# vkit-x/vkit

Hardware: AMD Instinct MI355X
Metric: Mpixels/s (2048^2 RGB, geo+photo chain) (higher is better)
Workload: dtype u8; 1 GPU; C3 fused chain: camera_cubic_curve remap (level 5) + gaussian_blur(sigma=1.0) + color_shift(37) + gaussion_noise(std=10.0, the numpy stream default_rng(5000 + i) drawn on the device inside every step), states built from the configs inside every step, 2048x2048x3 uint8, batch 256 per GPU; batch_per_gpu=256, image=2048x2048x3, noise_mode=tiles, states=built on the device from the configs inside every step (vkx_camera_states_dev), lanes=1

## Files before the change

### vkit_amd/csrc/fused.hip

```cpp
#include "vkx_internal.h"
#include "vkx_cell.h"
#include "vkx_color.h"

#include <float.h>
#include <memory>
#include <stdlib.h>
#include <string.h>

namespace {

constexpr int W = 64;
constexpr int RMAX = 3;
constexpr int NLDSCELL = 64;
#ifndef VKX_FUSED_NWAVES
#define VKX_FUSED_NWAVES 8
#endif
constexpr int NWAVES = VKX_FUSED_NWAVES;
constexpr int NTHREADS = 64 * NWAVES;
constexpr int ROWS_PER_WAVE = 8;
constexpr int WH = NWAVES * ROWS_PER_WAVE;
__host__ __device__ constexpr int tile_side(int R) { return (W - 2 * R) & ~3; }
__host__ __device__ constexpr int tile_height(int R) { return WH == W ? tile_side(R) : WH - 2 * R; }
#ifndef VKX_FUSED_CGROUP
#define VKX_FUSED_CGROUP 2
// ... 25 lines not shown
    int R;
    int hue_on, hue_delta;
    unsigned short kq[8];
    int streak_on, streak_step, streak_thickness, streak_dash, streak_dash_step, streak_dash_gap;
    int streak_vert, streak_hori, streak_copy;
    int streak_color[3];
    float streak_alpha;
    int n_elems, pad_;
    const uint2 *noise_table;
    int noise_tiled, noise_tiles, noise_slot;
    float noise_tiles_per_sample;
    const uint2 *noise_rows;
    struct Elem {
        const void *src;
        void *dst;
        ptrdiff_t sstride, dstride;
        int cn, is_f32;
    } el[4];
};

struct ElemPack {
    ItemDev::Elem el[4];
    int n;
};

struct TileRect {
    int x0, y0, x1, y1;
    __host__ __device__ bool empty() const { return x1 < x0 || y1 < y0; }
};
__host__ __device__ inline TileRect interior_rect(int dw, int dh, int R)
{
    const int Tw = tile_side(R), Th = tile_height(R);
    TileRect r;
    r.x0 = (R + Tw - 1) / Tw;
    r.y0 = (R + Th - 1) / Th;
    r.x1 = dw - W + R >= 0 ? (dw - W + R) / Tw : -1;
    r.y1 = dh - WH + R >= 0 ? (dh - WH + R) / Th : -1;
    return r;
}

struct TileBin {
    int rmin, cmin;
    int rmax1, cmax1;
};

struct CellR {
    int ex[4], edx[4];
    short vx[4], vy[4];
    int flags, pad;
};
static_assert(sizeof(CellR) == 56, "CellR mirrors the tail of CellC");

__device__ __forceinline__ int find_item(const int *__restrict__ prefix, int n, int v)
{
    int lo = 0, hi = n - 1;
    while (lo < hi) {
        const int mid = (lo + hi + 1) >> 1;
        if (prefix[mid] <= v) lo = mid; else hi = mid - 1;
    }
    return lo;
}

constexpr int kLocalBins = 1024;

__global__ void __launch_bounds__(256) k_chain_setup(const ItemDev *__restrict__ items, const int *__restrict__ cell_prefix,
                                                     int n_items, int total_cells, int slots,
                                                     vkc::CellC *__restrict__ cells, TileBin *__restrict__ bins,
                                                     int *__restrict__ deferred )
{
    __shared__ int lbins[kLocalBins * 4];
// ... 436 lines not shown
                        px += ax + (step ? bx : 0);
                        py += ay + (step ? by : 0);
                    }
                } else {
                    const double h6 = lch[kk * 9 + 6], h7 = lch[kk * 9 + 7];
                    for (int s = k0; s <= k1; s++) {
                        const bool inside = (unsigned)(px - lox) < (unsigned)nx_ && (unsigned)(py - loy) < (unsigned)ny_;
                        if (inside && !(fma(1.0, 1.0, fma(h7, (double)(py + wy0), h6 * (double)(px + wx0))) == 0))
                            atomicMax(own + py * P_ + px, tag);
                        const bool step = err < 0;
                        err += step ? up : down;
                        px += ax + (step ? bx : 0);
                        py += ay + (step ? by : 0);
                    }
                }
            }
        }
        __syncthreads();
        if (phase_limit == 1) return;

        if (!INTERIOR && nc > NLDSCELL) {
            load_chunk(0, NLDSCELL);
            __syncthreads();
        }

        const int gx = wx0 + lane;
        const bool colok = INTERIOR || (gx >= cx0 && gx < cx1);
        int srcl[2 * RMAX + 1];
#pragma unroll
        for (int i = 0; i < 2 * RMAX + 1; i++) {
            int s = (R > 0 && i < K) ? (INTERIOR ? lane + i - R : vkd::reflect101(gx + i - R, dw) - wx0) : lane;
            srcl[i] = min(max(s, 0), W - 1) << 2;
        }
        const unsigned fast_xlim = (unsigned)max(sw - 2, 0), fast_ylim = (unsigned)max(sh - 1, 0);
        const double fxd = (double)gx;
        const bool exact_div = __builtin_amdgcn_readfirstlane(*lflag) != 0;
        for (int g0 = 0; g0 < ROWS_PER_WAVE; g0 += CGROUP) {
            int X[CGROUP], Y[CGROUP];
            bool rowok[CGROUP];
#pragma unroll
            for (int u = 0; u < CGROUP; u++) {
                const int ly = wave * ROWS_PER_WAVE + g0 + u;
                const int gy = wy0 + ly;
                rowok[u] = INTERIOR || (gy >= cy0 && gy < cy1);
                X[u] = 0; Y[u] = 0;
                if (rowok[u] && colok) {
                    const uint32_t o = own[ly * P_ + lane];
                    if (o != 0) {
                        const int k = (int)o - 1;
                        double h[8];
                        if (INTERIOR || k < NLDSCELL) {
                            lds_cdouble_t hp = (lds_cdouble_t)(lch + __umul24(k, 9));
                            asm volatile("" : "+v"(hp));
#pragma unroll
                            for (int j = 0; j < 8; j++) h[j] = hp[j];
                        } else {
                            const vkc::CellC VKX_GLOBAL *gc =
                                (const vkc::CellC VKX_GLOBAL *)(gcell + (r0 + div_small(k, ncol, rcp_ncol)) * cw + (c0 + k - div_small(k, ncol, rcp_ncol) * ncol));
#pragma unroll
                            for (int j = 0; j < 8; j++) h[j] = gc->H[j];
                        }
                        const double fy = (double)gy;
                        const double nx = fma(h[2], 1.0, fma(h[1], fy, h[0] * fxd));
                        const double ny = fma(h[5], 1.0, fma(h[4], fy, h[3] * fxd));
                        const double de = fma(1.0, 1.0, fma(h[7], fy, h[6] * fxd));
                        float qxf, qyf;
                        if (exact_div || !div_pair_f32_fast(nx, ny, de, qxf, qyf)) {
                            double qx, qy;
                            div_pair(nx, ny, de, qx, qy);
                            X[u] = vkd::cv_round((float)qx * 32.f);
                            Y[u] = vkd::cv_round((float)qy * 32.f);
                        } else {
                            X[u] = cvt_i32_sat(rintf(qxf * 32.f));
                            Y[u] = cvt_i32_sat(rintf(qyf * 32.f));
                        }
                    }
                }
            }
            if constexpr (KIND == 3) {
#pragma unroll
// ... 77 lines not shown
                    const uint32_t o0 = __umul24((uint32_t)sy, (uint32_t)sstride) + __umul24((uint32_t)sx, 3u);
                    ta[u] = *(const u64_u1 VKX_GLOBAL *)(src + (size_t)o0);
                    tb[u] = *(const u64_u1 VKX_GLOBAL *)(src + (size_t)(o0 + (uint32_t)sstride));
                }
            }
            uint32_t prb[CGROUP], pg[CGROUP];
#pragma unroll
            for (int u = 0; u < CGROUP; u++) {
                prb[u] = 0; pg[u] = 0;
                if (!rowok[u]) continue;
                if (colok) {
                    const int fx = X[u] & 31, fy = Y[u] & 31;
                    if (fast[u]) {
                        const uint32_t wx = (uint32_t)(32 - fx) | ((uint32_t)fx << 24);
                        const uint32_t t0 = (uint32_t)ta[u], t1 = (uint32_t)(ta[u] >> 32), b0 = (uint32_t)tb[u], b1 = (uint32_t)(tb[u] >> 32);
                        const uint32_t ar = __builtin_amdgcn_udot4(t0, wx, 0u, false);
                        const uint32_t ag = __builtin_amdgcn_udot4(__builtin_amdgcn_alignbyte(t1, t0, 1), wx, 0u, false);
                        const uint32_t ab = __builtin_amdgcn_udot4(__builtin_amdgcn_alignbyte(t1, t0, 2), wx, 0u, false);
                        const uint32_t br = __builtin_amdgcn_udot4(b0, wx, 0u, false);
                        const uint32_t bg = __builtin_amdgcn_udot4(__builtin_amdgcn_alignbyte(b1, b0, 1), wx, 0u, false);
                        const uint32_t bb = __builtin_amdgcn_udot4(__builtin_amdgcn_alignbyte(b1, b0, 2), wx, 0u, false);
                        const uint32_t wy0 = (uint32_t)(32 - fy), wy1 = (uint32_t)fy;
                        const uint32_t r = mad_u24(br, wy1, mad_u24_cs(ar, wy0, 512u)) >> 10;
                        const uint32_t g = mad_u24(bg, wy1, mad_u24_cs(ag, wy0, 512u)) >> 10;
                        const uint32_t b = mad_u24(bb, wy1, mad_u24_cs(ab, wy0, 512u)) >> 10;
                        prb[u] = r | (b << 16);
                        pg[u] = g;
                    } else {
                        rim_sample_rgb(src, sh, sw, sstride, X[u], Y[u], prb[u], pg[u]);
                    }
                }
            }
            static_assert(CGROUP == 2, "phase D works on the window-row pair of one iteration");
            const int ly0 = wave * ROWS_PER_WAVE + g0;
            if (!(rowok[0] || rowok[1])) continue;
            if (R > 0) {
                const uint32_t gg = pg[0] | (pg[1] << 16);
                uint32_t a0 = 0, a1 = 0, ag = 0;
#pragma unroll
                for (int i = 0; i < 2 * RMAX + 1; i++) {
                    if (i < K) {
                        uint32_t v0 = prb[0], v1 = prb[1], vg = gg;
                        if (!(INTERIOR && RC >= 0 && i == RC)) {
                            v0 = (uint32_t)__builtin_amdgcn_ds_bpermute(srcl[i], (int)prb[0]);
                            v1 = (uint32_t)__builtin_amdgcn_ds_bpermute(srcl[i], (int)prb[1]);
                            vg = (uint32_t)__builtin_amdgcn_ds_bpermute(srcl[i], (int)gg);
                        }
                        a0 = mad_u24_ks(kq[i], v0, a0);
                        a1 = mad_u24_ks(kq[i], v1, a1);
                        ag = mad_u24_ks(kq[i], vg, ag);
                    }
                }
                uint32_t *pl = own + ly0 * P_ + lane;
                pl[0] = __builtin_amdgcn_perm(a1, a0, 0x05040100u);
                pl[64] = ag;
                pl[128] = __builtin_amdgcn_perm(a1, a0, 0x07060302u);
            } else {
#pragma unroll
                for (int u = 0; u < CGROUP; u++)
                    if (rowok[u]) own[(ly0 + u) * P_ + lane] = (prb[u] & 0xffu) | (pg[u] << 8) | (prb[u] & 0xff0000u);
            }
        }
        if constexpr (KIND == 3) return;
        __syncthreads();
        if (phase_limit == 2) return;

    }
// ... 703 lines not shown
```

### vkit_amd/csrc/nprand.hip

```cpp
#include "vkx_internal.h"
#include "np_ziggurat.h"
#include "vkx_host_tables.h"

#include <stddef.h>
#include <string.h>
#include <algorithm>

namespace {

typedef unsigned __int128 u128;
#define VKX_GLOBAL __attribute__((address_space(1)))

#ifndef VKX_NP_ROUNDS
#define VKX_NP_ROUNDS 48
#endif
constexpr int kRounds = VKX_NP_ROUNDS;
static_assert(kRounds % 2 == 0 && kRounds >= 2 && kRounds <= 64, "rounds per tile");
constexpr int kTile = 64 * kRounds;
constexpr double kNorR = 3.6541528853610087963519472518;
constexpr double kNorInvR = 0.27366123732975827203338247596;

#define PCG_MULT VKX_PCG_MULT
using vkx_host_tables::JumpTabs;

struct NpTabs {
    JumpTabs jump;
    uint64_t ki[256], wi[256], fi[256];
};

struct NpJob {
    uint64_t state[2], inc[2];
    uint64_t c64[2];
    uint64_t c128[2];
    long long n;
    long long tile_base;
    int n_tiles;
    int kind, cn;
    double loc, scale;
    double margin;
    double cdf[3];
    const uint8_t *src;
    void *dst;
    int16_t *rec;
    uint2 *table;
};

struct TileInfo {
    uint32_t count0, out0;
    uint64_t start0, emit0;
};
constexpr uint32_t kIrregular = 0x80000000u;
constexpr uint32_t kParkOver = 0x40000000u;
constexpr uint32_t kOutCarry = 0x3fffffffu;
constexpr uint32_t kFlagParkOver = 0x40000000u;
struct TilePlan {
    unsigned long long prefix;
    uint32_t c_in, count;
};

typedef uint32_t u32x4 __attribute__((ext_vector_type(4)));
struct FiC { double fi, c; };
__device__ __forceinline__ u128 mk128(const uint64_t *w) { return ((u128)w[1] << 64) | (u128)w[0]; }

__device__ __forceinline__ uint64_t pcg_out(u128 s)
{
    const uint64_t hi = (uint64_t)(s >> 64), lo = (uint64_t)s;
    const uint64_t x = hi ^ lo;
    const unsigned r = (unsigned)(hi >> 58);
    return (x >> r) | (x << ((64 - r) & 63));
}
struct LcgStride {
    uint32_t a0, a1, a2, a3;
    uint64_t c0, c1, c23;
};
__device__ __forceinline__ LcgStride lcg_stride(u128 a, u128 c)
{
    LcgStride k;
    k.a0 = (uint32_t)a; k.a1 = (uint32_t)(a >> 32); k.a2 = (uint32_t)(a >> 64); k.a3 = (uint32_t)(a >> 96);
    k.c0 = (uint32_t)c; k.c1 = (uint32_t)(c >> 32); k.c23 = (uint64_t)(c >> 64);
    return k;
}
__device__ __forceinline__ uint64_t mad_u64_u32_v(uint32_t a, uint32_t b, uint64_t c)
{
    uint64_t d, carry;
    asm("v_mad_u64_u32 %0, %1, %2, %3, %4" : "=v"(d), "=s"(carry) : "v"(a), "v"(b), "v"(c));
    return d;
}
__device__ __forceinline__ uint64_t mul_u64_u32_v(uint32_t a, uint32_t b)
{
    uint64_t d, carry;
    asm("v_mad_u64_u32 %0, %1, %2, %3, 0" : "=v"(d), "=s"(carry) : "v"(a), "v"(b));
    return d;
}
// ... 149 lines not shown
    const uint32_t base = lds_offset(flat);
    const uint32_t *pairs = (const uint32_t *)flat;
    uint32_t run = 0;
    constexpr int kBatch = 8;
    static_assert(kRounds % kBatch == 0 || kRounds < kBatch, "rounds per compaction batch");
#pragma unroll
    for (int r0 = 0; r0 < kRounds; r0 += kBatch) {
        uint32_t v[kBatch / 2];
#pragma unroll
        for (int j = 0; j < kBatch; j += 2)
            if (r0 + j < kRounds) v[j / 2] = pairs[32 * (r0 + j) + lane];
#pragma unroll
        for (int j = 0; j < kBatch; j++) {
            const int r = r0 + j;
            if (r >= kRounds) break;
            const uint32_t lo = (uint32_t)__builtin_amdgcn_readlane((int)m, r), hi = (uint32_t)__builtin_amdgcn_readlane((int)(m >> 32), r);
            const uint32_t rank = (uint32_t)__builtin_amdgcn_mbcnt_hi(hi, __builtin_amdgcn_mbcnt_lo(lo, run));
            const uint32_t addr = base + 2 * rank;
            const uint64_t mask = ((uint64_t)hi << 32) | lo;
            uint64_t saved;
            if (j & 1)
                asm volatile("s_mov_b64 %[sv], exec\n\ts_mov_b64 exec, %[m]\n\tds_write_b16_d16_hi %[a], %[v]\n\ts_mov_b64 exec, %[sv]"
                             : [sv] "=&s"(saved) : [m] "s"(mask), [a] "v"(addr), [v] "v"(v[j / 2]) : "memory");
            else
                asm volatile("s_mov_b64 %[sv], exec\n\ts_mov_b64 exec, %[m]\n\tds_write_b16 %[a], %[v]\n\ts_mov_b64 exec, %[sv]"
                             : [sv] "=&s"(saved) : [m] "s"(mask), [a] "v"(addr), [v] "v"(v[j / 2]) : "memory");
            run += (uint32_t)__builtin_popcountll(mask);
        }
    }
    __builtin_amdgcn_wave_barrier();
    return run;
}

__device__ __forceinline__ uint32_t park_index_b8(uint32_t pos) { return (pos & ~255u) | ((pos & 63u) << 2) | ((pos >> 6) & 3u); }

__device__ __forceinline__ uint32_t compact_tile_lds_b8(int8_t *flat, uint64_t m)
{
    const uint32_t lane = (uint32_t)__lane_id();
    const uint32_t base = lds_offset(flat);
    const uint32_t *quads = (const uint32_t *)flat;
    uint32_t run = 0;
    constexpr int kBatch = 8;
    static_assert(kRounds % kBatch == 0, "rounds per compaction batch");
#pragma unroll
    for (int r0 = 0; r0 < kRounds; r0 += kBatch) {
        uint32_t v[kBatch / 4];
#pragma unroll
        for (int j = 0; j < kBatch; j += 4) v[j / 4] = quads[16 * (r0 + j) + lane];
#pragma unroll
        for (int j = 0; j < kBatch; j++) {
            const int r = r0 + j;
            const uint32_t lo = (uint32_t)__builtin_amdgcn_readlane((int)m, r), hi = (uint32_t)__builtin_amdgcn_readlane((int)(m >> 32), r);
            const uint32_t addr = base + (uint32_t)__builtin_amdgcn_mbcnt_hi(hi, __builtin_amdgcn_mbcnt_lo(lo, run));
            const uint64_t mask = ((uint64_t)hi << 32) | lo;
            const uint32_t b = (j & 1) ? v[j / 4] >> 8 : v[j / 4];
            uint64_t saved;
            if (j & 2)
                asm volatile("s_mov_b64 %[sv], exec\n\ts_mov_b64 exec, %[m]\n\tds_write_b8_d16_hi %[a], %[v]\n\ts_mov_b64 exec, %[sv]"
                             : [sv] "=&s"(saved) : [m] "s"(mask), [a] "v"(addr), [v] "v"(b) : "memory");
            else
                asm volatile("s_mov_b64 %[sv], exec\n\ts_mov_b64 exec, %[m]\n\tds_write_b8 %[a], %[v]\n\ts_mov_b64 exec, %[sv]"
                             : [sv] "=&s"(saved) : [m] "s"(mask), [a] "v"(addr), [v] "v"(b) : "memory");
            run += (uint32_t)__builtin_popcountll(mask);
        }
    }
    __builtin_amdgcn_wave_barrier();
    return run;
}

typedef short s16x2 __attribute__((ext_vector_type(2)));
__device__ __forceinline__ uint32_t widen_b8_pair(uint32_t w, uint32_t sel)
{
    const uint32_t up = __builtin_amdgcn_perm(w, w, sel);
    s16x2 h;
    memcpy(&h, &up, 4);
    h = h >> (s16x2)8;
    uint32_t out;
    memcpy(&out, &h, 4);
    return out;
}

__device__ __attribute__((noinline)) double exp_f64_call(double y) { return exp(y); }

template <class Emit, int MODE>
__device__ void walk_tile(const NpJob &job, const JumpTabs &g_jump, const uint4 *__restrict__ zig , const FiC *__restrict__ fic ,
                          WaveWork<typename Emit::Park, MODE == kEmit || MODE == kCompact> &ws, u128 &s, u128 &s2, uint32_t c_in, long long prefix,
                          long long draw_base, typename Emit::Store VKX_GLOBAL *rec_val, uint64_t VKX_GLOBAL *rec_mask, void *emit_dst,
                          uint32_t &count_out, uint32_t &carry_out, uint64_t &start0, uint64_t &emit0, bool &has_tail, uint32_t &flags,
                          unsigned long long *draws_used)
{
    const int lane = __lane_id();
    const u128 inc = mk128(job.inc);
    constexpr bool kParkBytes = sizeof(typename Emit::Park) == 1;
    static_assert(!kParkBytes || MODE == kCompact, "bytes are parked by the compacting draw pass only");
    c_in = (uint32_t)__builtin_amdgcn_readfirstlane((int)c_in);
    prefix = (long long)rfl64((uint64_t)prefix);
    draw_base = (long long)rfl64((uint64_t)draw_base);
    uint32_t nev = 0;
    if (lane < kRounds) {
        ws.semit[lane] = 0;
        ws.slow[lane] = 0;
    }
    struct Draw {
        uint32_t hi, dlo, dhi;
        u32x4 e;
        double c;
    };
    uint32_t k_m20 = 0x000fffffu, k_exp = 0x43300000u, k_sgn = 0x80000000u;
    asm volatile("" : "+v"(k_m20), "+v"(k_exp), "+v"(k_sgn));
    auto lookup = [&](const u128 &st) {
        Draw d;
        const uint64_t hi = (uint64_t)(st >> 64), x = hi ^ (uint64_t)st;
        const uint32_t r = (uint32_t)(hi >> 58);
        const uint64_t v = (x >> ((r + 9) & 63)) | (x << ((55 - r) & 63));
        d.hi = (uint32_t)(v >> 32);
        d.dlo = (uint32_t)v;
        d.dhi = __builtin_amdgcn_bitop3_b32(d.hi, k_m20, k_exp, 0xea );
        const uint32_t off = (d.hi >> 19) & 0xff0u;
        d.e = *(const u32x4 *)((const char *)zig + off);
        if (MODE != kCount) d.c = *(const double *)((const char *)fic + off + offsetof(FiC, c));
        return d;
    };
    auto finish = [&](int r, const u128 &st, const Draw &d) -> typename Emit::Val {
        typename Emit::Val v = 0;
        if (MODE != kCount) {
            const double wi = __longlong_as_double((long long)(((uint64_t)d.e[3] << 32) | d.e[2]));
            const uint64_t xa = (uint64_t)__double_as_longlong(__builtin_fma(__longlong_as_double((long long)(((uint64_t)d.dhi << 32) | d.dlo)), wi, d.c));
            const uint32_t xs = __builtin_amdgcn_bitop3_b32(d.hi, k_sgn, (uint32_t)(xa >> 32), 0xea);
            const double x = __longlong_as_double((long long)(((uint64_t)xs << 32) | (uint32_t)xa));
            v = Emit::make(job, x, false, flags);
            if (MODE == kRecord) rec_val[64 * r + lane] = (typename Emit::Store)v;
            else if (MODE == kEmit) ws.val[r][lane] = (typename Emit::Store)v;
        }
        const bool slow_me = (((uint64_t)d.dhi << 32) | d.dlo) >= (((uint64_t)d.e[1] << 32) | d.e[0]);
        const uint64_t slow = __ballot(slow_me);
        if (slow) {
            if (slow_me) {
                const uint32_t slot = nev + (uint32_t)mbcnt64(slow);
                if (slot < (uint32_t)kEvCap) {
                    ws.ev_s[slot][0] = (uint64_t)st;
                    ws.ev_s[slot][1] = (uint64_t)(st >> 64);
                    ws.ev_pos[slot] = (uint16_t)(64 * r + lane);
                }
            }
            nev += (uint32_t)__builtin_popcountll(slow);
        }
        return v;
    };
    LcgStride stride128 = lcg_stride(mk128(g_jump.a128), mk128(job.c128));
    asm volatile("" : "+v"(stride128.a0), "+v"(stride128.a1), "+v"(stride128.a2), "+v"(stride128.a3));
    u128 sl = s, sl2 = s2;
#pragma unroll 2
    for (int r = 0; r < kRounds; r += 2) {
        const u128 sa = sl, sb = sl2;
        const Draw da = lookup(sa), db = lookup(sb);
        sl = lcg_step(sl, stride128);
        sl2 = lcg_step(sl2, stride128);
        const typename Emit::Val va = finish(r, sa, da);
        const typename Emit::Val vb = finish(r + 1, sb, db);
        if constexpr (MODE == kCompact && kParkBytes)
            ((uint16_t *)&ws.val[0][0])[128 * (r >> 2) + ((r >> 1) & 1) + 2 * lane] =
                (uint16_t)__builtin_amdgcn_perm((uint32_t)vb, (uint32_t)va, 0x0c0c0400u);
        else if constexpr (MODE == kCompact)
            ((uint32_t *)&ws.val[0][0])[32 * r + lane] = __builtin_amdgcn_perm((uint32_t)vb, (uint32_t)va, 0x05040100u);
    }
    s = sl;
    s2 = sl2;
    if (nev > (uint32_t)kEvCap) {
        flags |= VKX_NP_SHORT;
        nev = kEvCap;
    }
    __builtin_amdgcn_wave_barrier();
    if (MODE == kRecord) asm volatile("s_waitcnt vmcnt(0)" ::: "memory");
    has_tail = false;
#pragma unroll
    for (int q = 0; q < (kEvCap + 63) / 64; q++) {
        if ((uint32_t)(64 * q) >= nev) break;
        const uint32_t ev = 64 * q + lane;
        if (ev < nev) {
            const u128 se = ((u128)ws.ev_s[ev][1] << 64) | ws.ev_s[ev][0];
            const int pos = ws.ev_pos[ev];
            const uint64_t u = pcg_out(se);
            const int idx = (int)(u & 0xff);
            const uint64_t rabs = (u >> 9) & 0x000fffffffffffffull;
            uint32_t info;
            if (idx != 0) {
                double x = (__longlong_as_double((long long)(0x4330000000000000ull | rabs)) - 4503599627370496.0) *
                           __longlong_as_double(((long long)zig[idx].w << 32) | zig[idx].z);
                if (u & 0x100) x = -x;
                const double un = u2dbl(pcg_out(PCG_MULT * se + inc));
                const double f1 = fic[idx].fi, f0 = fic[idx - 1].fi;
                const double lhs = (f0 - f1) * un + f1;
                const double t = -0.5 * x;
                const double y = t * x;
                const float r32 = __builtin_amdgcn_exp2f((float)y * 1.44269504f);
                const float l32 = (float)lhs;
// ... 15 lines not shown
                    const uint64_t d1 = pcg_out(t);
                    t = PCG_MULT * t + inc;
                    const uint64_t d2 = pcg_out(t);
                    len += 2;
                    if constexpr (Emit::kFastTail) {
                        if (job.margin < 1.0) {
                            const double L1 = tail_log_est(d1), L2 = tail_log_est(d2);
                            const double xe = kNorInvR * L1, r2 = xe * xe;
                            const double diff = (L2 + L2) - r2;
                            const double bound = 2.0 * kTailEps + (kNorInvR * kNorInvR) * (2.0 * L1 * kTailEps + kTailEps * kTailEps) +
                                                 0x1p-30 * (1.0 + r2);
                            const bool decided = fabs(diff) > bound;
                            if (decided && diff < 0.0 && len <= 200) continue;
                            if (decided && diff > 0.0 && Emit::tail_proven(job, neg ? -(kNorR + xe) : kNorR + xe)) {
                                xx = xe;
                                inexact = false;
                                break;
                            }
                        }
                    }
                    const double u1 = u2dbl(d1), u2 = u2dbl(d2);
                    xx = -kNorInvR * log1p(-u1);
                    const double yy = -log1p(-u2);
                    const double l2 = yy + yy, r2 = xx * xx;
                    if (fabs(l2 - r2) <= r2 * 0x1p-40) flags |= VKX_NP_AMBIGUOUS;
                    if (l2 > r2 || len > 200) break;
                }
                if (len > 200) flags |= VKX_NP_SHORT;
                const double z = neg ? -(kNorR + xx) : kNorR + xx;
                if (MODE == kRecord) {
                    rec_val[pos] = (typename Emit::Store)Emit::make(job, z, inexact, flags);
                } else if constexpr (MODE == kCompact && kParkBytes) {
                    const int k = (int)Emit::make(job, z, inexact, flags);
                    (&ws.val[0][0])[park_index_b8(pos)] = (int8_t)k;
                    if (k != (int)(int8_t)k) flags |= kFlagParkOver;
                } else if (MODE == kCompact) {
                    (&ws.val[0][0])[park_index(pos)] = (typename Emit::Store)Emit::make(job, z, inexact, flags);
                } else if (MODE == kEmit) {
                    const typename Emit::Val v = Emit::make(job, z, inexact, flags);
                    uint64_t bits = 0;
                    memcpy(&bits, &v, sizeof v);
                    ws.ev_s[ev][0] = bits;
                }
                has_tail = true;
                info = len | 0x300u;
            }
            ws.ev_info[ev] = (uint16_t)info;
            atomicOr((unsigned long long *)&ws.slow[pos >> 6], 1ull << (pos & 63));
            if (info & 0x100u) atomicOr((unsigned long long *)&ws.semit[pos >> 6], 1ull << (pos & 63));
        }
    }
    __builtin_amdgcn_wave_barrier();
    has_tail = __ballot(has_tail) != 0;
    uint32_t P = 0xffffu, end = 0, info = 0;
    if ((uint32_t)lane < nev) {
        P = ws.ev_pos[lane];
        info = ws.ev_info[lane];
        end = P + (info & 0xffu);
    }
    uint64_t valid;
    uint32_t carry = c_in > (uint32_t)kTile ? c_in - kTile : 0u;
    if (nev <= 64) {
        const uint32_t prev_end = (uint32_t)__builtin_amdgcn_update_dpp((int)c_in, (int)end, 0x138 , 0xf, 0xf, false);
        const uint64_t live = nev == 64 ? ~0ull : ((1ull << nev) - 1);
        const uint64_t touch = __ballot((uint32_t)lane < nev && P < prev_end);
        valid = live;
        if (touch) {
// ... 30 lines not shown
        }
        __builtin_amdgcn_wave_barrier();
    } else {
        valid = 0;
        if (lane < kRounds) ws.cov()[lane] = 0;
        __builtin_amdgcn_wave_barrier();
        uint32_t cover_end = c_in;
        for (uint32_t e = 0; e < nev; e++) {
            const uint32_t pe = ws.ev_pos[e], ee = pe + (ws.ev_info[e] & 0xffu);
            if (pe < cover_end) continue;
            cover_end = ee;
            if (lane == 0)
                for (uint32_t q = pe + 1; q < ee && q < (uint32_t)kTile; q++) ws.cov()[q >> 6] |= 1ull << (q & 63);
        }
        if (cover_end > (uint32_t)kTile && cover_end - kTile > carry) carry = cover_end - kTile;
        __builtin_amdgcn_wave_barrier();
    }
    uint64_t my_mask = 0, my_starts = 0;
    if (lane < kRounds) {
        uint64_t cov = ws.cov()[lane];
        const uint32_t lo = 64u * lane;
        if (c_in > lo) cov |= c_in - lo >= 64 ? ~0ull : ((1ull << (c_in - lo)) - 1);
        const uint64_t slow = ws.slow[lane];
        my_starts = ~cov;
        my_mask = my_starts & (~slow | ws.semit[lane]);
    }
    start0 = rfl64(my_starts);
    emit0 = rfl64(my_mask);
    uint32_t count = (uint32_t)__builtin_popcountll(my_mask);
    count += (uint32_t)__builtin_amdgcn_update_dpp(0, (int)count, 0x118 , 0xf, 0xf, true);
    count += (uint32_t)__builtin_amdgcn_update_dpp(0, (int)count, 0x114 , 0xf, 0xf, true);
    count += (uint32_t)__builtin_amdgcn_update_dpp(0, (int)count, 0x112 , 0xf, 0xf, true);
    count += (uint32_t)__builtin_amdgcn_update_dpp(0, (int)count, 0x111 , 0xf, 0xf, true);
    {
        uint32_t total = (uint32_t)__builtin_amdgcn_readlane((int)count, 15);
        if (kRounds > 16) total += (uint32_t)__builtin_amdgcn_readlane((int)count, 31);
        if (kRounds > 32) total += (uint32_t)__builtin_amdgcn_readlane((int)count, 47);
        if (kRounds > 48) total += (uint32_t)__builtin_amdgcn_readlane((int)count, 63);
        count = total;
    }
    if (MODE == kEmit) {
        uint32_t done = 0, ebase = 0;
#pragma unroll 1
        for (int r = 0; r < kRounds; r++) {
            if (prefix + done >= job.n) break;
            const uint64_t emits = ((uint64_t)(uint32_t)__builtin_amdgcn_readlane((int)(my_mask >> 32), r) << 32) |
                                   (uint32_t)__builtin_amdgcn_readlane((int)my_mask, r);
            const uint64_t slow = rfl64(ws.slow[r]);
            const bool mine = (emits >> lane) & 1;
            const long long pos = prefix + done + mbcnt64(emits);
            if (mine && pos < job.n) {
                typename Emit::Val z = (typename Emit::Val)ws.val[r][lane];
                bool inexact = false;
                int len = 1;
                if ((slow >> lane) & 1) {
                    const uint32_t ev = ebase + (uint32_t)mbcnt64(slow);
                    const uint32_t einfo = ws.ev_info[ev];
                    len = (int)(einfo & 0xff);
                    if (einfo & 0x200u) {
                        const uint64_t bits = ws.ev_s[ev][0];
                        memcpy(&z, &bits, sizeof z);
                        inexact = true;
                    }
                }
                Emit::store(job, emit_dst, pos, z, inexact, flags);
                if (pos == job.n - 1)
                    __hip_atomic_store(draws_used, (unsigned long long)(draw_base + 64 * r + lane + len), __ATOMIC_RELAXED, __HIP_MEMORY_SCOPE_AGENT);
            }
            done += (uint32_t)__builtin_popcountll(emits);
            ebase += (uint32_t)__builtin_popcountll(slow);
        }
    }
    if (MODE == kRecord && lane < kRounds) rec_mask[lane] = my_mask;
    if constexpr (MODE == kCompact && kParkBytes) {
        static_assert(sizeof(typename Emit::Store) == 2, "compact records are int16");
        int8_t *flat = (int8_t *)&ws.val[0][0];
        const uint32_t total = compact_tile_lds_b8(flat, my_mask);
        const uint32_t groups = (total + 7) >> 3;
        const uint2 *f8 = (const uint2 *)flat;
        u32x4 VKX_GLOBAL *s16 = (u32x4 VKX_GLOBAL *)rec_val;
#pragma unroll
        for (int i = 0; i < kTile / 512; i++) {
            const uint32_t idx = (uint32_t)lane + 64u * i;
            if (idx < groups) {
                const uint2 b = f8[idx];
                u32x4 g;
                g[0] = widen_b8_pair(b.x, 0x010c000cu);
                g[1] = widen_b8_pair(b.x, 0x030c020cu);
                g[2] = widen_b8_pair(b.y, 0x010c000cu);
                g[3] = widen_b8_pair(b.y, 0x030c020cu);
                s16[idx] = g;
            }
        }
        __builtin_amdgcn_wave_barrier();
    } else if constexpr (MODE == kCompact) {
        static_assert(sizeof(typename Emit::Store) == 2, "compact records are int16");
        int16_t *flat = (int16_t *)&ws.val[0][0];
        const uint32_t total = compact_tile_lds(flat, my_mask);
        const uint32_t groups = (total + 7) >> 3;
        const u32x4 *f16 = (const u32x4 *)flat;
        u32x4 VKX_GLOBAL *s16 = (u32x4 VKX_GLOBAL *)rec_val;
#pragma unroll
        for (int i = 0; i < kTile / 512; i++) {
            const uint32_t idx = (uint32_t)lane + 64u * i;
            if (idx < groups) s16[idx] = f16[idx];
        }
        __builtin_amdgcn_wave_barrier();
    }
    count_out = count;
    carry_out = carry;
}
// ... 116 lines not shown
k_np_draw_compact(const NpJob *__restrict__ jobs, int n_jobs, long long total_tiles, long long run, const uint64_t *__restrict__ states,
                  TileInfo *__restrict__ info, vkx_np_result *__restrict__ results, const NpTabs *__restrict__ tabs)
{
    constexpr int kWaves = DrawShape<Emit>::kWaves;
    typedef WaveWork<typename Emit::Park, true> Work;
    struct Lds {
        uint4 zig[256];
        FiC fic[256];
        Work work[kWaves];
    };
    __shared__ Lds lds;
    uint4 *zig = lds.zig;
    FiC *fic = lds.fic;
    Work *work = lds.work;
    load_tables(zig, fic, tabs);
    const JumpTabs &g_jump = tabs->jump;
    const long long wave = (long long)blockIdx.x * kWaves + __builtin_amdgcn_readfirstlane((int)(threadIdx.x >> 6));
    const long long run_end = min(total_tiles, (wave + 1) * run);
    int j = 0;
    long long job_end = 0;
    u128 s = 0, s2 = 0;
    for (long long tile = wave * run; tile < run_end; tile++) {
        if (tile >= job_end) {
            j = job_of_tile(jobs, n_jobs, tile);
            job_end = jobs[j].tile_base + jobs[j].n_tiles;
            tile_lane_states(g_jump, jobs[j], mk128(&states[2 * tile]), s, s2);
        }
        const NpJob &job = jobs[j];
        uint32_t count, carry, flags = 0;
        uint64_t start0, emit0;
        bool has_tail;
        walk_tile<Emit, kCompact>(job, g_jump, zig, fic, work[threadIdx.x >> 6], s, s2, 0u, 0, 0,
                                  (int16_t VKX_GLOBAL *)(job.rec + (tile - job.tile_base) * kSlot), nullptr, nullptr,
                                  count, carry, start0, emit0, has_tail, flags, nullptr);
        const bool over = __ballot((flags & kFlagParkOver) != 0) != 0;
        flags &= ~kFlagParkOver;
        if (__lane_id() == 0) {
            TileInfo t;
            t.count0 = count; t.out0 = carry | (has_tail ? 0x80000000u : 0u) | (over ? kParkOver : 0u); t.start0 = start0; t.emit0 = emit0;
            info[tile] = t;
        }
        if (flags) atomicOr(&results[j].flags, flags);
    }
}

__global__ void __launch_bounds__(1024) k_np_resolve(const NpJob *__restrict__ jobs, const uint64_t *__restrict__ states,
                                                     const TileInfo *__restrict__ info_all, TilePlan *__restrict__ plan_all,
                                                     vkx_np_result *__restrict__ results, const NpTabs *__restrict__ tabs)
{
    __shared__ uint4 zig[256];
    __shared__ FiC fic[256];
    __shared__ WaveWork<int16_t, false> work[1];
    __shared__ unsigned long long part[1024];
    __shared__ uint32_t n_irregular;
    extern __shared__ uint64_t irregular[];
    const NpJob &job = jobs[blockIdx.x];
    const int T = job.n_tiles;
    const TileInfo *info = info_all + job.tile_base;
    TilePlan *plan = plan_all + job.tile_base;
    const uint64_t *st = states + 2 * job.tile_base;
    const int words = (T + 63) >> 6;
    if (threadIdx.x == 0) n_irregular = 0;
    load_tables(zig, fic, tabs);
    const JumpTabs &g_jump = tabs->jump;
    for (int w = threadIdx.x >> 6; w < words; w += 16) {
        const int j = w * 64 + (threadIdx.x & 63);
        bool bad = false;
// ... 322 lines not shown
                uint8_t *d = (uint8_t *)job.dst + e * cn;
                if (job.kind == VKX_NP_CHOICE3_U8) {
                    d[0] = (uint8_t)sel;
                } else {
                    const uint8_t *p = job.src + e * cn;
                    for (int k = 0; k < cn; k++) d[k] = sel == 1 ? 255 : (sel == 2 ? 0 : p[k]);
                }
            }
            s = a64 * s + c64;
        }
    }
    np_results_out(done, results, results_host, n_jobs);
}

__global__ void __launch_bounds__(256) k_np_tail_log_est(const uint64_t *__restrict__ draws, long long n, double *__restrict__ est)
{
    const long long i = (long long)blockIdx.x * 256 + threadIdx.x;
    if (i < n) est[i] = tail_log_est(draws[i]);
}

}

static int np_tables(vkx_ctx *ctx, const NpTabs **out)
{
    if (!ctx->np_tabs.ptr) {
        vkx_tables tab(ctx);
        int rc = tab.take(sizeof(NpTabs));
        if (rc) return rc;
        NpTabs *t = tab.at<NpTabs>(0);
        t->jump = vkx_host_tables::jump_tabs();
        memcpy(t->ki, kNpZigK, 2048);
        memcpy(t->wi, kNpZigW, 2048);
        memcpy(t->fi, kNpZigF, 2048);
        if ((rc = tab.copy_to(&ctx->np_tabs))) return rc;
    }
    *out = (const NpTabs *)ctx->np_tabs.ptr;
    return VKX_OK;
}

static long long np_tiles_for_n(long long n, bool uniform)
{
    const long long draws = uniform ? n : n + n / 45 + 4096;
    return (draws + kTile - 1) / kTile;
}
static long long np_tiles_for(const vkx_np_job &j, bool uniform) { return np_tiles_for_n(j.n, uniform); }

vkx_np_tiles_shape vkx_np_tiles_shape_of(long long n)
{
    vkx_np_tiles_shape s;
    s.n_tiles = np_tiles_for_n(n, false);
    s.slot_elems = kSlot;
    s.table_offset = 16;
    s.slots_offset = vkx_align256(16 + 8 * ((size_t)s.n_tiles + 1));
    s.bytes = s.slots_offset + (size_t)s.n_tiles * kSlot * 2;
    s.samples_per_tile = (double)kTile * 0.97850;
    return s;
}

VKX_EXPORT int vkx_np_tiles_layout(int64_t n, int64_t *n_tiles, int64_t *slot_elems, int64_t *table_offset, int64_t *slots_offset,
                                   int64_t *bytes)
{
    VKX_REQUIRE(n >= 1 && n <= 0x7fffffffLL, "1 .. 2^31 - 1 samples");
    const vkx_np_tiles_shape s = vkx_np_tiles_shape_of(n);
    if (n_tiles) *n_tiles = s.n_tiles;
    if (slot_elems) *slot_elems = s.slot_elems;
    if (table_offset) *table_offset = (int64_t)s.table_offset;
// ... 385 lines not shown
```

Before: 79030 Mpixels/s.

## Route border tiles through the interior kernel via reflected coordinates

Widens the interior tile rectangle so tiles touching the image border also take the INTERIOR path. Pixels outside the image get reflect101-mirrored coordinates, computed per lane for columns and through a readlane row table for rows, and these feed the owner lookup and the homography. For the bottom edge the row order within a wave is remapped. The aim is to avoid the slower non-interior path with its bounds checks for edge tiles. In exchange it adds index arithmetic, and correctness now depends on the mirrored coordinates and the remapped row order matching the old edge handling.

Measured after the change: 79480 Mpixels/s, median of 6. Within noise of the previous version (+0.6%).

```diff
diff --git a/vkit_amd/csrc/fused.hip b/vkit_amd/csrc/fused.hip
--- a/vkit_amd/csrc/fused.hip
+++ b/vkit_amd/csrc/fused.hip
@@ -81,10 +81,10 @@
 {
     const int Tw = tile_side(R), Th = tile_height(R);
     TileRect r;
-    r.x0 = (R + Tw - 1) / Tw;
-    r.y0 = (R + Th - 1) / Th;
-    r.x1 = dw - W + R >= 0 ? (dw - W + R) / Tw : -1;
-    r.y1 = dh - WH + R >= 0 ? (dh - WH + R) / Th : -1;
+    r.x0 = 0;
+    r.y0 = 0;
+    r.x1 = dw >= W ? (dw - W + 2 * R) / Tw : -1;
+    r.y1 = dh >= WH ? (dh - WH + 2 * R) / Th : -1;
     return r;
 }
 
@@ -587,20 +587,35 @@
             int s = (R > 0 && i < K) ? (INTERIOR ? lane + i - R : vkd::reflect101(gx + i - R, dw) - wx0) : lane;
             srcl[i] = min(max(s, 0), W - 1) << 2;
         }
+        const int agx = gx < 0 ? -gx : gx;
+        const int rgx = INTERIOR ? min(agx, 2 * (dw - 1) - agx) : gx;
+        const int rlx = rgx - wx0;
         const unsigned fast_xlim = (unsigned)max(sw - 2, 0), fast_ylim = (unsigned)max(sh - 1, 0);
-        const double fxd = (double)gx;
+        const double fxd = (double)rgx;
         const bool exact_div = __builtin_amdgcn_readfirstlane(*lflag) != 0;
+        int rowtab = 0;
+        if constexpr (INTERIOR) {
+            const int j = lane & (ROWS_PER_WAVE - 1), jp = j & ~(CGROUP - 1);
+            const int ly = wave * ROWS_PER_WAVE + (wy0 + WH > dh ? ROWS_PER_WAVE - CGROUP - jp : jp) + (j - jp);
+            const int wy = wy0 + ly, awy = wy < 0 ? -wy : wy;
+            rowtab = ly | ((min(awy, 2 * (dh - 1) - awy) - wy0) << 8);
+        }
         for (int g0 = 0; g0 < ROWS_PER_WAVE; g0 += CGROUP) {
-            int X[CGROUP], Y[CGROUP];
+            int X[CGROUP], Y[CGROUP], lyw[CGROUP];
             bool rowok[CGROUP];
 #pragma unroll
             for (int u = 0; u < CGROUP; u++) {
-                const int ly = wave * ROWS_PER_WAVE + g0 + u;
-                const int gy = wy0 + ly;
+                int ly = wave * ROWS_PER_WAVE + g0 + u, rly = ly;
+                if constexpr (INTERIOR) {
+                    const int e = __builtin_amdgcn_readlane(rowtab, g0 + u);
+                    ly = e & 0xff; rly = e >> 8;
+                }
+                lyw[u] = ly;
+                const int gy = wy0 + rly;
                 rowok[u] = INTERIOR || (gy >= cy0 && gy < cy1);
                 X[u] = 0; Y[u] = 0;
                 if (rowok[u] && colok) {
-                    const uint32_t o = own[ly * P_ + lane];
+                    const uint32_t o = own[rly * P_ + rlx];
                     if (o != 0) {
                         const int k = (int)o - 1;
                         double h[8];
@@ -744,7 +759,7 @@
                 }
             }
             static_assert(CGROUP == 2, "phase D works on the window-row pair of one iteration");
-            const int ly0 = wave * ROWS_PER_WAVE + g0;
+            const int ly0 = lyw[0];
             if (!(rowok[0] || rowok[1])) continue;
             if (R > 0) {
                 const uint32_t gg = pg[0] | (pg[1] << 16);
```

## Replace per-round LDS byte compaction with table-driven 8-byte group squeeze

Applied to the files above, without the earlier changes.

Replaces the serial per-round compaction of parked int8 noise values (one masked LDS byte write per round) with a per-lane squeeze: each lane handles an 8-byte group, looks up a precomputed byte-permute selector for its keep mask, and writes the kept bytes at an offset built from prefix counts stored per round. The park layout becomes linear, and per-round offsets come from an extra DPP scan. This cuts the number of serialized readlane/mbcnt/exec-swap steps, at the cost of a 256-entry global selector table lookup and eight ballots per pass.

Measured after the change: 78560 Mpixels/s before, 78730 Mpixels/s after, median of 2. No clear change (+0.2%).

```diff
diff --git a/vkit_amd/csrc/nprand.hip b/vkit_amd/csrc/nprand.hip
--- a/vkit_amd/csrc/nprand.hip
+++ b/vkit_amd/csrc/nprand.hip
@@ -26,7 +26,20 @@
 struct NpTabs {
     JumpTabs jump;
     uint64_t ki[256], wi[256], fi[256];
+    uint2 squeeze[256];
 };
+
+inline uint2 squeeze_selectors(uint32_t mb)
+{
+    uint32_t sel[2] = {0x0c0c0c0cu, 0x0c0c0c0cu};
+    int k = 0;
+    for (uint32_t b = 0; b < 8; b++)
+        if ((mb >> b) & 1) {
+            sel[k >> 2] = (sel[k >> 2] & ~(0xffu << (8 * (k & 3)))) | (b << (8 * (k & 3)));
+            k++;
+        }
+    return make_uint2(sel[0], sel[1]);
+}
 
 struct NpJob {
     uint64_t state[2], inc[2];
@@ -59,6 +72,7 @@
 };
 
 typedef uint32_t u32x4 __attribute__((ext_vector_type(4)));
+typedef uint32_t u32x2 __attribute__((ext_vector_type(2)));
 struct FiC { double fi, c; };
 __device__ __forceinline__ u128 mk128(const uint64_t *w) { return ((u128)w[1] << 64) | (u128)w[0]; }
 
@@ -274,41 +288,54 @@
     return run;
 }
 
-__device__ __forceinline__ uint32_t park_index_b8(uint32_t pos) { return (pos & ~255u) | ((pos & 63u) << 2) | ((pos >> 6) & 3u); }
-
-__device__ __forceinline__ uint32_t compact_tile_lds_b8(int8_t *flat, uint64_t m)
-{
-    const uint32_t lane = (uint32_t)__lane_id();
-    const uint32_t base = lds_offset(flat);
-    const uint32_t *quads = (const uint32_t *)flat;
-    uint32_t run = 0;
-    constexpr int kBatch = 8;
-    static_assert(kRounds % kBatch == 0, "rounds per compaction batch");
+typedef uint8_t __attribute__((may_alias)) u8_alias;
+typedef uint32_t __attribute__((may_alias)) u32_alias;
+typedef u32x2 __attribute__((may_alias)) u32x2_alias;
+
+#define VKX_DS_WRITE_UNDER(OP, MASK, ADDR, VAL, ...)                                                                                  \
+    asm volatile("s_mov_b64 %[sv], exec\n\ts_mov_b64 exec, %[m]\n\t" OP " %[a], %[v]" __VA_ARGS__ "\n\ts_mov_b64 exec, %[sv]"                  \
+                 : [sv] "=&s"(saved) : [m] "s"(MASK), [a] "v"(ADDR), [v] "v"(VAL) : "memory")
+
+__device__ __forceinline__ void squeeze_tile_lds_b8(int8_t *flat, const uint64_t *masks, const uint64_t *place, const u32x2 VKX_GLOBAL *sel)
+{
+    constexpr int kPasses = kTile / 512;
+    static_assert(kTile % 512 == 0, "whole passes of 64 groups");
+    uint32_t lane = (uint32_t)__lane_id();
+    asm volatile("" : "+v"(lane));
+    const uint32_t sub = lane >> 3;
+    const uint64_t below = (1ull << (8 * (lane & 7))) - 1;
+    uint32_t mb[kPasses];
+    u32x2 s[kPasses];
 #pragma unroll
-    for (int r0 = 0; r0 < kRounds; r0 += kBatch) {
-        uint32_t v[kBatch / 4];
+    for (int p = 0; p < kPasses; p++) mb[p] = ((const u8_alias *)masks)[64 * p + lane];
 #pragma unroll
-        for (int j = 0; j < kBatch; j += 4) v[j / 4] = quads[16 * (r0 + j) + lane];
+    for (int p = 0; p < kPasses; p++) {
+        asm("" : "+v"(mb[p]));
+        s[p] = *(const u32x2 VKX_GLOBAL *)((const char VKX_GLOBAL *)sel + (mb[p] << 3));
+    }
 #pragma unroll
-        for (int j = 0; j < kBatch; j++) {
-            const int r = r0 + j;
-            const uint32_t lo = (uint32_t)__builtin_amdgcn_readlane((int)m, r), hi = (uint32_t)__builtin_amdgcn_readlane((int)(m >> 32), r);
-            const uint32_t addr = base + (uint32_t)__builtin_amdgcn_mbcnt_hi(hi, __builtin_amdgcn_mbcnt_lo(lo, run));
-            const uint64_t mask = ((uint64_t)hi << 32) | lo;
-            const uint32_t b = (j & 1) ? v[j / 4] >> 8 : v[j / 4];
-            uint64_t saved;
-            if (j & 2)
-                asm volatile("s_mov_b64 %[sv], exec\n\ts_mov_b64 exec, %[m]\n\tds_write_b8_d16_hi %[a], %[v]\n\ts_mov_b64 exec, %[sv]"
-                             : [sv] "=&s"(saved) : [m] "s"(mask), [a] "v"(addr), [v] "v"(b) : "memory");
-            else
-                asm volatile("s_mov_b64 %[sv], exec\n\ts_mov_b64 exec, %[m]\n\tds_write_b8 %[a], %[v]\n\ts_mov_b64 exec, %[sv]"
-                             : [sv] "=&s"(saved) : [m] "s"(mask), [a] "v"(addr), [v] "v"(b) : "memory");
-            run += (uint32_t)__builtin_popcountll(mask);
-        }
+    for (int p = 0; p < kPasses; p++) {
+        const uint64_t before = masks[8 * p + sub] & below;
+        uint32_t o = (uint32_t)__builtin_popcount((uint32_t)before) + ((const u32_alias *)place)[2 * (8 * p + sub)];
+        asm("" : "+v"(o));
+        o += (uint32_t)__builtin_popcount((uint32_t)(before >> 32));
+        const u32x2 b = ((const u32x2_alias *)flat)[64 * p + lane];
+        const uint32_t n = (uint32_t)__builtin_popcount(mb[p]);
+        const uint32_t lo = __builtin_amdgcn_perm(b.y, b.x, s[p].x), hi = __builtin_amdgcn_perm(b.y, b.x, s[p].y);
+        const uint32_t lo1 = lo >> 8, hi1 = hi >> 8;
+        uint64_t saved;
+        VKX_DS_WRITE_UNDER("ds_write_b8", __ballot(n > 0u), o, lo);
+        VKX_DS_WRITE_UNDER("ds_write_b8", __ballot(n > 1u), o, lo1, " offset:1");
+        VKX_DS_WRITE_UNDER("ds_write_b8_d16_hi", __ballot(n > 2u), o, lo, " offset:2");
+        VKX_DS_WRITE_UNDER("ds_write_b8_d16_hi", __ballot(n > 3u), o, lo1, " offset:3");
+        VKX_DS_WRITE_UNDER("ds_write_b8", __ballot(n > 4u), o, hi, " offset:4");
+        VKX_DS_WRITE_UNDER("ds_write_b8", __ballot(n > 5u), o, hi1, " offset:5");
+        VKX_DS_WRITE_UNDER("ds_write_b8_d16_hi", __ballot(n > 6u), o, hi, " offset:6");
+        VKX_DS_WRITE_UNDER("ds_write_b8_d16_hi", __ballot(n > 7u), o, hi1, " offset:7");
     }
     __builtin_amdgcn_wave_barrier();
-    return run;
-}
+}
+#undef VKX_DS_WRITE_UNDER
 
 typedef short s16x2 __attribute__((ext_vector_type(2)));
 __device__ __forceinline__ uint32_t widen_b8_pair(uint32_t w, uint32_t sel)
@@ -329,12 +356,13 @@
                           WaveWork<typename Emit::Park, MODE == kEmit || MODE == kCompact> &ws, u128 &s, u128 &s2, uint32_t c_in, long long prefix,
                           long long draw_base, typename Emit::Store VKX_GLOBAL *rec_val, uint64_t VKX_GLOBAL *rec_mask, void *emit_dst,
                           uint32_t &count_out, uint32_t &carry_out, uint64_t &start0, uint64_t &emit0, bool &has_tail, uint32_t &flags,
-                          unsigned long long *draws_used)
+                          unsigned long long *draws_used, const u32x2 VKX_GLOBAL *squeeze  = nullptr)
 {
     const int lane = __lane_id();
     const u128 inc = mk128(job.inc);
     constexpr bool kParkBytes = sizeof(typename Emit::Park) == 1;
     static_assert(!kParkBytes || MODE == kCompact, "bytes are parked by the compacting draw pass only");
+    if constexpr (kParkBytes) __builtin_assume_separate_storage(&job, &ws);
     c_in = (uint32_t)__builtin_amdgcn_readfirstlane((int)c_in);
     prefix = (long long)rfl64((uint64_t)prefix);
     draw_base = (long long)rfl64((uint64_t)draw_base);
@@ -400,10 +428,10 @@
         sl2 = lcg_step(sl2, stride128);
         const typename Emit::Val va = finish(r, sa, da);
         const typename Emit::Val vb = finish(r + 1, sb, db);
-        if constexpr (MODE == kCompact && kParkBytes)
-            ((uint16_t *)&ws.val[0][0])[128 * (r >> 2) + ((r >> 1) & 1) + 2 * lane] =
-                (uint16_t)__builtin_amdgcn_perm((uint32_t)vb, (uint32_t)va, 0x0c0c0400u);
-        else if constexpr (MODE == kCompact)
+        if constexpr (MODE == kCompact && kParkBytes) {
+            ws.val[r][lane] = (int8_t)va;
+            ws.val[r + 1][lane] = (int8_t)vb;
+        } else if constexpr (MODE == kCompact)
             ((uint32_t *)&ws.val[0][0])[32 * r + lane] = __builtin_amdgcn_perm((uint32_t)vb, (uint32_t)va, 0x05040100u);
     }
     s = sl;
@@ -485,7 +513,7 @@
                     rec_val[pos] = (typename Emit::Store)Emit::make(job, z, inexact, flags);
                 } else if constexpr (MODE == kCompact && kParkBytes) {
                     const int k = (int)Emit::make(job, z, inexact, flags);
-                    (&ws.val[0][0])[park_index_b8(pos)] = (int8_t)k;
+                    (&ws.val[0][0])[pos] = (int8_t)k;
                     if (k != (int)(int8_t)k) flags |= kFlagParkOver;
                 } else if (MODE == kCompact) {
                     (&ws.val[0][0])[park_index(pos)] = (typename Emit::Store)Emit::make(job, z, inexact, flags);
@@ -582,7 +610,17 @@
     count += (uint32_t)__builtin_amdgcn_update_dpp(0, (int)count, 0x114 , 0xf, 0xf, true);
     count += (uint32_t)__builtin_amdgcn_update_dpp(0, (int)count, 0x112 , 0xf, 0xf, true);
     count += (uint32_t)__builtin_amdgcn_update_dpp(0, (int)count, 0x111 , 0xf, 0xf, true);
-    {
+    if constexpr (MODE == kCompact && kParkBytes) {
+        const uint32_t own = (uint32_t)__builtin_popcountll(my_mask);
+        count += (uint32_t)__builtin_amdgcn_update_dpp(0, (int)count, 0x142 , 0xa, 0xf, false);
+        count += (uint32_t)__builtin_amdgcn_update_dpp(0, (int)count, 0x143 , 0xc, 0xf, false);
+        if (lane < kRounds) {
+            ws.slow[lane] = my_mask;
+            ws.semit[lane] = lds_offset(&ws.val[0][0]) + count - own;
+        }
+        __builtin_amdgcn_wave_barrier();
+        count = (uint32_t)__builtin_amdgcn_readlane((int)count, 63);
+    } else {
         uint32_t total = (uint32_t)__builtin_amdgcn_readlane((int)count, 15);
         if (kRounds > 16) total += (uint32_t)__builtin_amdgcn_readlane((int)count, 31);
         if (kRounds > 32) total += (uint32_t)__builtin_amdgcn_readlane((int)count, 47);
@@ -625,8 +663,8 @@
     if constexpr (MODE == kCompact && kParkBytes) {
         static_assert(sizeof(typename Emit::Store) == 2, "compact records are int16");
         int8_t *flat = (int8_t *)&ws.val[0][0];
-        const uint32_t total = compact_tile_lds_b8(flat, my_mask);
-        const uint32_t groups = (total + 7) >> 3;
+        squeeze_tile_lds_b8(flat, ws.slow, ws.semit, squeeze);
+        const uint32_t groups = (count + 7) >> 3;
         const uint2 *f8 = (const uint2 *)flat;
         u32x4 VKX_GLOBAL *s16 = (u32x4 VKX_GLOBAL *)rec_val;
 #pragma unroll
@@ -809,7 +847,7 @@
         bool has_tail;
         walk_tile<Emit, kCompact>(job, g_jump, zig, fic, work[threadIdx.x >> 6], s, s2, 0u, 0, 0,
                                   (int16_t VKX_GLOBAL *)(job.rec + (tile - job.tile_base) * kSlot), nullptr, nullptr,
-                                  count, carry, start0, emit0, has_tail, flags, nullptr);
+                                  count, carry, start0, emit0, has_tail, flags, nullptr, (const u32x2 VKX_GLOBAL *)tabs->squeeze);
         const bool over = __ballot((flags & kFlagParkOver) != 0) != 0;
         flags &= ~kFlagParkOver;
         if (__lane_id() == 0) {
@@ -1198,6 +1236,7 @@
         memcpy(t->ki, kNpZigK, 2048);
         memcpy(t->wi, kNpZigW, 2048);
         memcpy(t->fi, kNpZigF, 2048);
+        for (uint32_t mb = 0; mb < 256; mb++) t->squeeze[mb] = squeeze_selectors(mb);
         if ((rc = tab.copy_to(&ctx->np_tabs))) return rc;
     }
     *out = (const NpTabs *)ctx->np_tabs.ptr;
```
